# amorim-cleison/sign-language-nlp

Measured on AMD Instinct MI355X. Metric: train seq/s (batch=50,len=48), higher is better.
Workload: dtype bf16x3; 1 GPU; cfg2: Transformer train step E512 H8 N6 F512 batch 50 len 48 |src| 3000 |tgt| 202 dropout 0.1, fwd+CE+bwd+clip(0.5)+SGD(m=.9); launch=eager stream launches (auto: timed both in 9 untimed pre-warmup steps + warmup), per_gpu=independent fit (grid shard)

## Files before the change

sign-language-nlp_amd/csrc/attention.hip:

```cpp
#include "common.hpp"
#include "launch.hpp"

namespace slnlp {

constexpr int SMAX = 64;
constexpr int DCH = 64;
constexpr int TLD = 68;

typedef __attribute__((ext_vector_type(8))) __bf16 bf16x8;
typedef __attribute__((ext_vector_type(4))) short s16x4;
typedef __attribute__((ext_vector_type(8))) short s16x8;
typedef __attribute__((ext_vector_type(4))) float f32x4;

constexpr int ALD = 72;
constexpr int ATILE = SMAX * ALD;
constexpr int MFMA_DH = 64;

__device__ __forceinline__ void fetch_tile(const float* __restrict__ src, long ld, int B, int b, int S, int col0,
                                           int dc, int tid, float4 (&r)[4]) {
#pragma unroll
    for (int u = 0; u < 4; ++u) {
        const int idx = tid + 256 * u, s = idx >> 4, c = (idx & 15) << 2;
        const bool ok = s < S && c < dc;
        r[u] = *reinterpret_cast<const float4*>(src + ((long)(ok ? s : 0) * B + b) * ld + col0 + (ok ? c : 0));
// ... 27 lines not shown
    const s16x8 v = {v0[0], v0[1], v0[2], v0[3], v1[0], v1[1], v1[2], v1[3]};
    return __builtin_bit_cast(bf16x8, v);
}
__device__ __forceinline__ f32x4 mfma3(bf16x8 ah, bf16x8 al, bf16x8 bh, bf16x8 bl, f32x4 c) {
    c = __builtin_amdgcn_mfma_f32_16x16x32_bf16(al, bh, c, 0, 0, 0);
    c = __builtin_amdgcn_mfma_f32_16x16x32_bf16(ah, bl, c, 0, 0, 0);
    return __builtin_amdgcn_mfma_f32_16x16x32_bf16(ah, bh, c, 0, 0, 0);
}
__device__ __forceinline__ unsigned keep_mask8(const DropKey& key, unsigned row0, unsigned col, unsigned thr) {
    unsigned m = 0;
    if ((row0 & 3u) == 0u) {
        const uint4 bits = dropout_bits8(key, row0 >> 2, drop_cc(col));
#pragma unroll
        for (int h = 0; h < 2; ++h)
#pragma unroll
            for (int r = 0; r < 4; ++r) m |= (pick_lot(bits, h, r) >= thr ? 1u : 0u) << (4 * h + r);
    } else {
#pragma unroll
        for (int h = 0; h < 2; ++h)
#pragma unroll
            for (int r = 0; r < 4; ++r) m |= (dropout_keep(key, row0 + r, col + 16 * h, thr) ? 1u : 0u) << (4 * h + r);
    }
    return m;
}
__device__ __forceinline__ void put_planes(unsigned short* __restrict__ T, int off, float v) {
    unsigned short h, l;
    split_bf16(v, h, l);
    T[off] = h;
    T[ATILE + off] = l;
}

__device__ __forceinline__ void store_rows_via_lds(unsigned short* __restrict__ T, const f32x4 (&o)[4], int wave, int lane, int S, int dc,
                                                   const PlaneOut& po, long row_stride, long col0, int B, int b) {
    const int jc = lane & 15, i0 = wave * 16 + ((lane >> 4) << 2);
#pragma unroll
    for (int n = 0; n < 4; ++n)
#pragma unroll
        for (int r = 0; r < 4; ++r) put_planes(T, (i0 + r) * ALD + 16 * n + jc, o[n][r]);
    asm volatile("s_waitcnt lgkmcnt(0)" ::: "memory");
    __builtin_amdgcn_wave_barrier();
#pragma unroll
    for (int pass = 0; pass < 2; ++pass) {
        const int row = wave * 16 + pass * 8 + (lane >> 3), c8 = (lane & 7) << 3;
        if (row < S && c8 < dc) {
            const uint4 vh = *reinterpret_cast<const uint4*>(T + row * ALD + c8), vl = *reinterpret_cast<const uint4*>(T + ATILE + row * ALD + c8);
            const long at = ((long)row * B + b) * row_stride + col0 + c8;
// ... 139 lines not shown
    const unsigned long long* __restrict__ rng, PlaneOut po) {
    extern __shared__ __attribute__((aligned(16))) float smem[];
    unsigned short* TQ = reinterpret_cast<unsigned short*>(smem);
    unsigned short* TK = TQ + 2 * ATILE;
    unsigned short* TO = TQ + 4 * ATILE;
    unsigned short* TV = TQ + 6 * ATILE;
    const int tid = threadIdx.x, lane = tid & 63, wave = tid >> 6;
    const int b = blockIdx.x / H, h = blockIdx.x % H, E = H * dh;
    const long ld = 3L * E;
    const int jc = lane & 15, i0 = wave * 16 + ((lane >> 4) << 2);
    const long prow0 = ((long)b * H + h) * S + i0;
    const int nch = (dh + MFMA_DH - 1) / MFMA_DH;
    unsigned short* TS = nch > 1 ? TQ + 8 * ATILE : TO;

    float pr[4][4];
#pragma unroll
    for (int n = 0; n < 4; ++n)
#pragma unroll
        for (int r = 0; r < 4; ++r) {
            const int j = 16 * n + jc;
            const bool ok = (i0 + r) < S && j < S;
            pr[n][r] = probs[ok ? (prow0 + r) * S + j : 0];
        }
    f32x4 acc[4];
#pragma unroll
    for (int n = 0; n < 4; ++n) acc[n] = f32x4{0.f, 0.f, 0.f, 0.f};
    float4 rq[4], rk[4];
    for (int ch = 0; ch < nch; ++ch) {
        const int d0 = ch * MFMA_DH, dc = dh - d0 < MFMA_DH ? dh - d0 : MFMA_DH;
        float4 ro[4], rv[4];
        fetch_tile(dctx, E, B, b, S, h * dh + d0, dc, tid, ro);
        fetch_tile(qkv, ld, B, b, S, 2 * E + h * dh + d0, dc, tid, rv);
        if (nch == 1) {
            fetch_tile(qkv, ld, B, b, S, h * dh, dc, tid, rq);
            fetch_tile(qkv, ld, B, b, S, E + h * dh, dc, tid, rk);
        }
        if (ch > 0) __syncthreads();
        stash_tile(TO, S, dc, tid, ro);
        stash_tile(TV, S, dc, tid, rv);
        __syncthreads();
        const int nk = (dc + 31) >> 5;
        for (int kk = 0; kk < nk; ++kk) {
            const bf16x8 ah = frag_rows(TO, wave * 16, kk, lane), al = frag_rows(TO + ATILE, wave * 16, kk, lane);
#pragma unroll
            for (int n = 0; n < 4; ++n)
                acc[n] = mfma3(ah, al, frag_rows(TV, 16 * n, kk, lane), frag_rows(TV + ATILE, 16 * n, kk, lane), acc[n]);
        }
    }
    if (nch == 1) {
        stash_tile(TQ, S, dh, tid, rq);
        stash_tile(TK, S, dh, tid, rk);
    }
    const float scale = rsqrtf((float)dh), inv_keep = 1.f / (1.f - drop_p);
    float ds[4][4], pd[4][4];
    {
        unsigned keep[4] = {15u, 15u, 15u, 15u};
        if (drop_p > 0.f) {
            const DropKey dkey = dropout_key(rng, drop_site);
#pragma unroll
            for (int np = 0; np < 2; ++np) {
                if (32 * np + jc >= S || i0 >= S) continue;
                const unsigned m = keep_mask8(dkey, (unsigned)prow0, (unsigned)(32 * np + jc), drop_thr);
                keep[2 * np] = m & 15u;
                keep[2 * np + 1] = m >> 4;
            }
        }
#pragma unroll
        for (int r = 0; r < 4; ++r) {
            float dp[4], s = 0.f;
#pragma unroll
            for (int n = 0; n < 4; ++n) {
                const bool ok = (i0 + r) < S && (16 * n + jc) < S;
                const float p = ok ? pr[n][r] : 0.f;
                const bool k = (keep[n] >> r) & 1u;
                pr[n][r] = p;
                dp[n] = drop_p > 0.f ? (k ? acc[n][r] * inv_keep : 0.f) : acc[n][r];
                pd[n][r] = drop_p > 0.f ? (k ? p * inv_keep : 0.f) : p;
                s += dp[n] * p;
            }
            s = row16_sum(s);
#pragma unroll
            for (int n = 0; n < 4; ++n) ds[n][r] = pr[n][r] * (dp[n] - s) * scale;
        }
    }
    __syncthreads();
#pragma unroll
    for (int n = 0; n < 4; ++n)
#pragma unroll
        for (int r = 0; r < 4; ++r) {
// ... 363 lines not shown
```

sign-language-nlp_amd/csrc/attention_mem.hip:

```cpp
#include <stddef.h>

#include "common.hpp"
#include "launch.hpp"

namespace slnlp {


__device__ __forceinline__ int xcd_local(int i, int nb) { return (nb & 7) == 0 ? (i & 7) * (nb >> 3) + (i >> 3) : i; }

template <class F>
__device__ __forceinline__ void row_dots(const float* __restrict__ v, const float* __restrict__ mem, int B, int b, int S, int E, int lane,
                                         int wave, F&& put) {
    for (int s0 = wave; s0 < S; s0 += 16) {
        float a[4] = {0.f, 0.f, 0.f, 0.f};
#pragma unroll
        for (int u = 0; u < 4; ++u) {
            const int s = s0 + 4 * u;
            if (s < S) {
                const float* mr = mem + ((long)s * B + b) * E;
                for (int e = lane * 4; e < E; e += 256) {
                    const float4 m4 = *reinterpret_cast<const float4*>(mr + e), q4 = *reinterpret_cast<const float4*>(v + e);
                    a[u] += q4.x * m4.x + q4.y * m4.y + q4.z * m4.z + q4.w * m4.w;
                }
            }
        }
#pragma unroll
        for (int u = 0; u < 4; ++u) {
            const float r = wave_sum(a[u]);
            if (lane == 0 && s0 + 4 * u < S) put(s0 + 4 * u, r);
        }
    }
}

__device__ __forceinline__ void xmem_fwd_body(const float* __restrict__ qk, const float* __restrict__ mem, const float* __restrict__ bv,
                                              int B, int S, int H, int dh, float* __restrict__ mbar_out, float* __restrict__ psum_out,
                                              float* __restrict__ probs, float* __restrict__ ctx0, float drop_p, unsigned drop_thr,
                                              int drop_site, const unsigned long long* __restrict__ rng) {
    extern __shared__ __attribute__((aligned(16))) float xm_lds[];
    const int tid = threadIdx.x, lane = tid & 63, wave = tid >> 6;
    const int bh = xcd_local(blockIdx.x, gridDim.x), b = bh / H, h = bh % H, E = H * dh;
    float* qv = xm_lds;
    float* sc = qv + E;
    float* ps = sc + S;
    for (int e = tid * 4; e < E; e += 1024) *reinterpret_cast<float4*>(qv + e) = *reinterpret_cast<const float4*>(qk + (long)bh * E + e);
    __syncthreads();
    const float scale = rsqrtf((float)dh), inv_keep = 1.f / (1.f - drop_p);
    row_dots(qv, mem, B, b, S, E, lane, wave, [&](int s_, float r) { sc[s_] = r * scale; });
    __syncthreads();
    if (wave == 0) {
        float m = -INFINITY;
        for (int s = lane; s < S; s += 64) m = fmaxf(m, sc[s]);
        m = wave_max(m);
        float sum = 0.f;
        for (int s = lane; s < S; s += 64) sum += expf(sc[s] - m);
        sum = wave_sum(sum);
        float tot = 0.f;
        for (int s = lane; s < S; s += 64) {
            float p = expf(sc[s] - m) / sum;
            probs[(long)bh * S + s] = p;
            if (drop_p > 0.f) p = dropout_keep(rng, drop_site, (unsigned)bh, (unsigned)s, drop_thr) ? p * inv_keep : 0.f;
            sc[s] = p;
            tot += p;
        }
        tot = wave_sum(tot);
        if (lane == 0) {
            ps[0] = tot;
            psum_out[bh] = tot;
        }
    }
    __syncthreads();
    for (int e = tid * 4; e < E; e += 1024) {
        float4 a = make_float4(0.f, 0.f, 0.f, 0.f);
#pragma unroll 16
        for (int s = 0; s < S; ++s) {
            const float p = sc[s];
            const float4 m4 = *reinterpret_cast<const float4*>(mem + ((long)s * B + b) * E + e);
            a.x += p * m4.x; a.y += p * m4.y; a.z += p * m4.z; a.w += p * m4.w;
        }
        *reinterpret_cast<float4*>(mbar_out + (long)bh * E + e) = a;
    }
    for (int j = tid; j < dh; j += 256) ctx0[(long)b * E + h * dh + j] = bv[h * dh + j] * ps[0];
}
SLNLP_ZKERNEL(xmem_fwd_kernel, 256, xmem_fwd_body)

__device__ __forceinline__ void xmem_bwd_body(const float* __restrict__ mem, const float* __restrict__ bv, const float* __restrict__ probs,
                                              const float* __restrict__ psum, const float* __restrict__ dmbar,
                                              const float* __restrict__ dctx, int B, int S, int H, int dh, float* __restrict__ dsc_out,
                                              float* __restrict__ dqk_out, float* __restrict__ dcp, float drop_p, unsigned drop_thr,
                                              int drop_site, const unsigned long long* __restrict__ rng) {
    extern __shared__ __attribute__((aligned(16))) float xm_lds[];
    const int tid = threadIdx.x, lane = tid & 63, wave = tid >> 6;
    const int bh = xcd_local(blockIdx.x, gridDim.x), b = bh / H, h = bh % H, E = H * dh;
    float* dmb = xm_lds;
    float* t = dmb + E;
    float* cc = t + S;
    const float ps = psum[bh];
    for (int e = tid * 4; e < E; e += 1024) *reinterpret_cast<float4*>(dmb + e) = *reinterpret_cast<const float4*>(dmbar + (long)bh * E + e);
    if (wave == 0) {
        float c = 0.f;
        for (int j = lane; j < dh; j += 64) {
            const float g = dctx[(long)b * E + h * dh + j];
            c += g * bv[h * dh + j];
            dcp[(long)b * E + h * dh + j] = g * ps;
        }
        c = wave_sum(c);
        if (lane == 0) cc[0] = c;
    }
    __syncthreads();
    row_dots(dmb, mem, B, b, S, E, lane, wave, [&](int s_, float r) { t[s_] = r + cc[0]; });
    __syncthreads();
    const float scale = rsqrtf((float)dh), inv_keep = 1.f / (1.f - drop_p);
    if (wave == 0) {
        float dot = 0.f;
        for (int s = lane; s < S; s += 64) {
            float dp = t[s];
            if (drop_p > 0.f) dp = dropout_keep(rng, drop_site, (unsigned)bh, (unsigned)s, drop_thr) ? dp * inv_keep : 0.f;
            t[s] = dp;
            dot += probs[(long)bh * S + s] * dp;
        }
        dot = wave_sum(dot);
        for (int s = lane; s < S; s += 64) {
            const float v = probs[(long)bh * S + s] * (t[s] - dot) * scale;
            t[s] = v;
            dsc_out[(long)bh * S + s] = v;
        }
    }
    __syncthreads();
    for (int e = tid * 4; e < E; e += 1024) {
        float4 a = make_float4(0.f, 0.f, 0.f, 0.f);
#pragma unroll 16
        for (int s = 0; s < S; ++s) {
            const float w = t[s];
            const float4 m4 = *reinterpret_cast<const float4*>(mem + ((long)s * B + b) * E + e);
            a.x += w * m4.x; a.y += w * m4.y; a.z += w * m4.z; a.w += w * m4.w;
        }
        *reinterpret_cast<float4*>(dqk_out + (long)bh * E + e) = a;
    }
}
SLNLP_ZKERNEL(xmem_bwd_kernel, 256, xmem_bwd_body)

constexpr int XMEM_MAX_HEADS = 64;

constexpr int DMEM_ROWS = 8;
__device__ __forceinline__ void dmem_stage(const float* __restrict__ probs, const float* __restrict__ dsc, int b, int h, int s_, int S, int H,
                                           float drop_p, unsigned drop_thr, int drop_site, const unsigned long long* __restrict__ rng,
                                           float& p, float& d) {
    const long bh = (long)b * H + h;
    p = 0.f;
    d = 0.f;
    if (s_ < S) {
        p = probs[bh * S + s_];
        if (drop_p > 0.f) p = dropout_keep(rng, drop_site, (unsigned)bh, (unsigned)s_, drop_thr) ? p / (1.f - drop_p) : 0.f;
        d = dsc[bh * S + s_];
    }
}
constexpr int DMEM_HEADS = 2;
__device__ __forceinline__ void dmem_add_heads(float4 (&a)[DMEM_ROWS], const float* __restrict__ dmbar, const float* __restrict__ qk,
                                               const float* ph, const float* dh_, int ld, int b, int H, int E, int e, int set, int sets) {
    const int ni = (DMEM_ROWS + sets - 1) / sets;
    for (int h0 = 0; h0 < H; h0 += DMEM_HEADS) {
        float4 g[DMEM_HEADS], k[DMEM_HEADS];
#pragma unroll
        for (int u = 0; u < DMEM_HEADS; ++u) {
            const long bh = (long)b * H + (h0 + u < H ? h0 + u : H - 1);
            g[u] = *reinterpret_cast<const float4*>(dmbar + bh * E + e);
            k[u] = *reinterpret_cast<const float4*>(qk + bh * E + e);
        }
#pragma unroll
        for (int u = 0; u < DMEM_HEADS; ++u) {
            if (h0 + u >= H) break;
#pragma unroll
            for (int i = 0; i < DMEM_ROWS; ++i) {
                if (i >= ni) break;
                const int r = set + i * sets;
                const bool ok = r < DMEM_ROWS;
                const float p = ok ? ph[r * ld + h0 + u] : 0.f, d = ok ? dh_[r * ld + h0 + u] : 0.f;
                a[i].x += p * g[u].x + d * k[u].x; a[i].y += p * g[u].y + d * k[u].y; a[i].z += p * g[u].z + d * k[u].z; a[i].w += p * g[u].w + d * k[u].w;
            }
        }
    }
}
__device__ __forceinline__ void dmem_colsum(const float* __restrict__ dcp, int B, int E, int c, float* __restrict__ dbv) {
    if (c >= E) return;
    float a = 0.f;
#pragma unroll 8
    for (int r = 0; r < B; ++r) a += dcp[(long)r * E + c];
    dbv[c] = a;
}

__device__ __forceinline__ void xmem_dmem_body(const float* __restrict__ probs, const float* __restrict__ dsc, const float* __restrict__ dmbar,
                                               const float* __restrict__ qk, int B, int S, int H, int E, float* __restrict__ dmem,
                                               int accumulate, float drop_p, unsigned drop_thr, int drop_site,
                                               const unsigned long long* __restrict__ rng, const float* __restrict__ dcp,
                                               float* __restrict__ dbv) {
    __shared__ float ph[DMEM_ROWS][XMEM_MAX_HEADS], dh_[DMEM_ROWS][XMEM_MAX_HEADS];
    const int chunks = (S + DMEM_ROWS - 1) / DMEM_ROWS, tid = threadIdx.x;
    if ((int)blockIdx.x >= chunks * B) {
        dmem_colsum(dcp, B, E, ((int)blockIdx.x - chunks * B) * 256 + tid, dbv);
        return;
    }
    const int b = blockIdx.x / chunks, s0 = (blockIdx.x % chunks) * DMEM_ROWS;
    for (int i = tid; i < DMEM_ROWS * H; i += 256) {
        const int r = i / H, h = i - r * H;
        float p, d;
        dmem_stage(probs, dsc, b, h, s0 + r, S, H, drop_p, drop_thr, drop_site, rng, p, d);
        ph[r][h] = p;
        dh_[r][h] = d;
    }
    __syncthreads();
    const int per = E >> 2, sets = per >= 256 ? 1 : 256 / per;
    const int set = sets == 1 ? 0 : tid / per, c0 = sets == 1 ? tid : tid - set * per;
    if (set >= sets) return;
    for (int e = c0 * 4; e < E; e += (sets == 1 ? 1024 : E)) {
        float4 a[DMEM_ROWS];
#pragma unroll
        for (int i = 0; i < DMEM_ROWS; ++i) {
            const int r = set + i * sets, s_ = s0 + r;
            a[i] = make_float4(0.f, 0.f, 0.f, 0.f);
            if (accumulate && r < DMEM_ROWS && s_ < S) a[i] = *reinterpret_cast<const float4*>(dmem + ((long)s_ * B + b) * E + e);
        }
        dmem_add_heads(a, dmbar, qk, &ph[0][0], &dh_[0][0], XMEM_MAX_HEADS, b, H, E, e, set, sets);
#pragma unroll
        for (int i = 0; i < DMEM_ROWS; ++i) {
            const int r = set + i * sets, s_ = s0 + r;
            if (r < DMEM_ROWS && s_ < S) *reinterpret_cast<float4*>(dmem + ((long)s_ * B + b) * E + e) = a[i];
        }
    }
}
SLNLP_ZKERNEL(xmem_dmem_kernel, 256, xmem_dmem_body)

constexpr int DMEM_STAGE_LAYERS = 8;
template <class T>
__device__ __forceinline__ T* dmem_ptr(T* p) {
    const unsigned long long v = (unsigned long long)p;
    const unsigned lo = __builtin_amdgcn_readfirstlane((unsigned)v), hi = __builtin_amdgcn_readfirstlane((unsigned)(v >> 32));
    return as_global((T*)(((unsigned long long)hi << 32) | lo));
}
__device__ __forceinline__ void xmem_dmem_all_body(const XmemDmemLayer* __restrict__ tab, int N, int B, int S, int H, int E,
                                                   float* __restrict__ dmem, float drop_p, unsigned drop_thr,
                                                   const unsigned long long* __restrict__ rng) {
    extern __shared__ __attribute__((aligned(16))) float xm_lds[];
    const int chunks = (S + DMEM_ROWS - 1) / DMEM_ROWS, tid = threadIdx.x;
    if ((int)blockIdx.x >= chunks * B) {
        const int cb = (E + 255) / 256, i = (int)blockIdx.x - chunks * B, l = i / cb;
        if (l < N) dmem_colsum(dmem_ptr(tab[l].dcp), B, E, (i - l * cb) * 256 + tid, dmem_ptr(tab[l].dbv));
        return;
    }
    const int b = blockIdx.x / chunks, s0 = (blockIdx.x % chunks) * DMEM_ROWS;
    const int per = E >> 2, sets = per >= 256 ? 1 : 256 / per;
    const int set = sets == 1 ? 0 : tid / per, c0 = sets == 1 ? tid : tid - set * per, e = c0 * 4;
    const bool active = set < sets && e < E;
    const int lf = DMEM_ROWS * H, wave = __builtin_amdgcn_readfirstlane(tid >> 6), lane = tid & 63;
    float4 a[DMEM_ROWS];
#pragma unroll
    for (int i = 0; i < DMEM_ROWS; ++i) a[i] = make_float4(0.f, 0.f, 0.f, 0.f);
    for (int l1 = N; l1 > 0; l1 -= DMEM_STAGE_LAYERS) {
        const int n = l1 < DMEM_STAGE_LAYERS ? l1 : DMEM_STAGE_LAYERS;
        if (l1 != N) __syncthreads();
        for (int j = wave; j < n; j += 4) {
            const XmemDmemLayer L = tab[l1 - 1 - j];
            const float* __restrict__ probs = dmem_ptr(L.probs);
            const float* __restrict__ dsc = dmem_ptr(L.dsc);
            for (int i = lane; i < lf; i += 64) {
                const int r = i / H, h = i - r * H;
                float p, d;
                dmem_stage(probs, dsc, b, h, s0 + r, S, H, drop_p, drop_thr, L.drop_site, rng, p, d);
                xm_lds[2 * j * lf + i] = p;
                xm_lds[(2 * j + 1) * lf + i] = d;
            }
        }
        __syncthreads();
        if (active)
            for (int j = 0; j < n; ++j) {
                const XmemDmemLayer L = tab[l1 - 1 - j];
                dmem_add_heads(a, dmem_ptr(L.dmbar), dmem_ptr(L.qk), xm_lds + 2 * j * lf, xm_lds + (2 * j + 1) * lf, H, b, H, E, e, set, sets);
            }
    }
    if (!active) return;
#pragma unroll
    for (int i = 0; i < DMEM_ROWS; ++i) {
        const int r = set + i * sets, s_ = s0 + r;
        if (r < DMEM_ROWS && s_ < S) *reinterpret_cast<float4*>(dmem + ((long)s_ * B + b) * E + e) = a[i];
    }
}
SLNLP_ZKERNEL(xmem_dmem_all_kernel, 256, xmem_dmem_all_body)

__device__ __forceinline__ void xmem_colsum_body(const float* __restrict__ in, int R, int C, float* __restrict__ out) {
    const int c = blockIdx.x * 256 + threadIdx.x;
    if (c >= C) return;
// ... 33 lines not shown
#pragma unroll
        for (int u = 0; u < RU; ++u)
#pragma unroll
            for (int hp = 0; hp < HP; ++hp) {
                const float r = wave_sum(a[u][hp]);
                if (lane == 0 && s0 + 4 * u < S) put(hp, s0 + 4 * u, r);
            }
    }
}

__device__ __forceinline__ int xm_head_floats(int S, int E) { return E + ((S + 3) & ~3) + 4; }

template <int HP>
__device__ __forceinline__ void xmem_fwd_multi_body(const float* __restrict__ qk, const float* __restrict__ mem, const float* __restrict__ bv,
                                                    int B, int S, int H, int dh, float* __restrict__ mbar_out, float* __restrict__ psum_out,
                                                    float* __restrict__ probs, float* __restrict__ ctx0, float drop_p, unsigned drop_thr,
                                                    int drop_site, const unsigned long long* __restrict__ rng) {
    extern __shared__ __attribute__((aligned(16))) float xm_lds[];
    const int tid = threadIdx.x, lane = tid & 63, wave = tid >> 6;
    const int E = H * dh, groups = H / HP;
    const int wg = xcd_local(blockIdx.x, gridDim.x), b = wg / groups, h0 = (wg % groups) * HP;
    const int hf = xm_head_floats(S, E), sp = (S + 3) & ~3;
    float* heads = xm_lds;
    for (int i = tid * 4; i < HP * E; i += 1024) {
        const int hp = i / E, e = i - hp * E;
        *reinterpret_cast<float4*>(heads + (long)hp * hf + e) = *reinterpret_cast<const float4*>(qk + ((long)b * H + h0 + hp) * E + e);
    }
    __syncthreads();
    const float scale = rsqrtf((float)dh), inv_keep = 1.f / (1.f - drop_p);
    row_dots_multi<HP>(heads, hf, mem, B, b, S, E, lane, wave, [&](int hp, int s_, float r) { heads[(long)hp * hf + E + s_] = r * scale; });
    __syncthreads();
    for (int hp = wave; hp < HP; hp += 4) {
        float* sc = heads + (long)hp * hf + E;
        const long bh = (long)b * H + h0 + hp;
        float m = -INFINITY;
        for (int s_ = lane; s_ < S; s_ += 64) m = fmaxf(m, sc[s_]);
        m = wave_max(m);
        float sum = 0.f;
        for (int s_ = lane; s_ < S; s_ += 64) sum += expf(sc[s_] - m);
        sum = wave_sum(sum);
        float tot = 0.f;
        for (int s_ = lane; s_ < S; s_ += 64) {
            float p = expf(sc[s_] - m) / sum;
            probs[bh * S + s_] = p;
            if (drop_p > 0.f) p = dropout_keep(rng, drop_site, (unsigned)bh, (unsigned)s_, drop_thr) ? p * inv_keep : 0.f;
            sc[s_] = p;
            tot += p;
        }
        tot = wave_sum(tot);
        if (lane == 0) {
            sc[sp] = tot;
            psum_out[bh] = tot;
        }
    }
    __syncthreads();
    for (int e = tid * 4; e < E; e += 1024) {
        float4 a[HP];
#pragma unroll
        for (int hp = 0; hp < HP; ++hp) a[hp] = make_float4(0.f, 0.f, 0.f, 0.f);
#pragma unroll 8
        for (int s_ = 0; s_ < S; ++s_) {
            const float4 m4 = *reinterpret_cast<const float4*>(mem + ((long)s_ * B + b) * E + e);
#pragma unroll
            for (int hp = 0; hp < HP; ++hp) {
                const float p = heads[(long)hp * hf + E + s_];
                a[hp].x += p * m4.x; a[hp].y += p * m4.y; a[hp].z += p * m4.z; a[hp].w += p * m4.w;
            }
        }
// ... 10 lines not shown
                                                 const unsigned long long* rng) {
    xmem_fwd_multi_body<2>(qk, mem, bv, B, S, H, dh, mbar_out, psum_out, probs, ctx0, drop_p, drop_thr, drop_site, rng);
}
__device__ __forceinline__ void xmem_fwd_h4_body(const float* qk, const float* mem, const float* bv, int B, int S, int H, int dh, float* mbar_out,
                                                 float* psum_out, float* probs, float* ctx0, float drop_p, unsigned drop_thr, int drop_site,
                                                 const unsigned long long* rng) {
    xmem_fwd_multi_body<4>(qk, mem, bv, B, S, H, dh, mbar_out, psum_out, probs, ctx0, drop_p, drop_thr, drop_site, rng);
}
SLNLP_ZKERNEL(xmem_fwd_h2_kernel, 256, xmem_fwd_h2_body)
SLNLP_ZKERNEL(xmem_fwd_h4_kernel, 256, xmem_fwd_h4_body)

template <int HP>
__device__ __forceinline__ void xmem_bwd_multi_body(const float* __restrict__ mem, const float* __restrict__ bv, const float* __restrict__ probs,
                                                    const float* __restrict__ psum, const float* __restrict__ dmbar,
                                                    const float* __restrict__ dctx, int B, int S, int H, int dh, float* __restrict__ dsc_out,
                                                    float* __restrict__ dqk_out, float* __restrict__ dcp, float drop_p, unsigned drop_thr,
                                                    int drop_site, const unsigned long long* __restrict__ rng) {
    extern __shared__ __attribute__((aligned(16))) float xm_lds[];
    const int tid = threadIdx.x, lane = tid & 63, wave = tid >> 6;
    const int E = H * dh, groups = H / HP;
    const int wg = xcd_local(blockIdx.x, gridDim.x), b = wg / groups, h0 = (wg % groups) * HP;
    const int hf = xm_head_floats(S, E), sp = (S + 3) & ~3;
    float* heads = xm_lds;
    for (int i = tid * 4; i < HP * E; i += 1024) {
        const int hp = i / E, e = i - hp * E;
        *reinterpret_cast<float4*>(heads + (long)hp * hf + e) = *reinterpret_cast<const float4*>(dmbar + ((long)b * H + h0 + hp) * E + e);
    }
    for (int hp = wave; hp < HP; hp += 4) {
        const int h = h0 + hp;
        const float ps = psum[(long)b * H + h];
        float c = 0.f;
        for (int j = lane; j < dh; j += 64) {
            const float g = dctx[(long)b * E + h * dh + j];
            c += g * bv[h * dh + j];
            dcp[(long)b * E + h * dh + j] = g * ps;
        }
        c = wave_sum(c);
        if (lane == 0) heads[(long)hp * hf + E + sp] = c;
    }
    __syncthreads();
    row_dots_multi<HP>(heads, hf, mem, B, b, S, E, lane, wave,
                       [&](int hp, int s_, float r) { heads[(long)hp * hf + E + s_] = r + heads[(long)hp * hf + E + sp]; });
    __syncthreads();
    const float scale = rsqrtf((float)dh), inv_keep = 1.f / (1.f - drop_p);
    for (int hp = wave; hp < HP; hp += 4) {
        float* t = heads + (long)hp * hf + E;
        const long bh = (long)b * H + h0 + hp;
        float dot = 0.f;
        for (int s_ = lane; s_ < S; s_ += 64) {
            float dp = t[s_];
            if (drop_p > 0.f) dp = dropout_keep(rng, drop_site, (unsigned)bh, (unsigned)s_, drop_thr) ? dp * inv_keep : 0.f;
            t[s_] = dp;
            dot += probs[bh * S + s_] * dp;
        }
        dot = wave_sum(dot);
        for (int s_ = lane; s_ < S; s_ += 64) {
            const float v = probs[bh * S + s_] * (t[s_] - dot) * scale;
            t[s_] = v;
            dsc_out[bh * S + s_] = v;
        }
    }
    __syncthreads();
    for (int e = tid * 4; e < E; e += 1024) {
        float4 a[HP];
#pragma unroll
        for (int hp = 0; hp < HP; ++hp) a[hp] = make_float4(0.f, 0.f, 0.f, 0.f);
#pragma unroll 8
        for (int s_ = 0; s_ < S; ++s_) {
            const float4 m4 = *reinterpret_cast<const float4*>(mem + ((long)s_ * B + b) * E + e);
#pragma unroll
            for (int hp = 0; hp < HP; ++hp) {
                const float w = heads[(long)hp * hf + E + s_];
                a[hp].x += w * m4.x; a[hp].y += w * m4.y; a[hp].z += w * m4.z; a[hp].w += w * m4.w;
            }
        }
#pragma unroll
        for (int hp = 0; hp < HP; ++hp) *reinterpret_cast<float4*>(dqk_out + ((long)b * H + h0 + hp) * E + e) = a[hp];
    }
}
__device__ __forceinline__ void xmem_bwd_h2_body(const float* mem, const float* bv, const float* probs, const float* psum, const float* dmbar,
                                                 const float* dctx, int B, int S, int H, int dh, float* dsc_out, float* dqk_out, float* dcp,
                                                 float drop_p, unsigned drop_thr, int drop_site, const unsigned long long* rng) {
    xmem_bwd_multi_body<2>(mem, bv, probs, psum, dmbar, dctx, B, S, H, dh, dsc_out, dqk_out, dcp, drop_p, drop_thr, drop_site, rng);
}
// ... 130 lines not shown
```

sign-language-nlp_amd/csrc/elementwise.hip:

```cpp
#include "common.hpp"
#include "launch.hpp"
#include "layernorm_row.hpp"

namespace slnlp {

__device__ __forceinline__ void embed_fwd_body(const long* __restrict__ ids, long ld_ids, int B, int S,
                                                        int E, int V, const float* __restrict__ table,
                                                        const float* __restrict__ pe, float* __restrict__ out,
                                                        float scale, float drop_p, unsigned drop_thr, int drop_site,
                                                        const unsigned long long* __restrict__ rng, long nan_idx,
                                                        PlaneOut po, unsigned char* __restrict__ keep_mask) {
    const int e4 = E >> 2;
    const long total = (long)B * S * e4;
    const float ik = 1.f / (1.f - drop_p);
    for (long idx = blockIdx.x * 256L + threadIdx.x; idx < total; idx += (long)gridDim.x * 256) {
        const int m = (int)(idx / e4), c = (int)(idx % e4) * 4;
        const int s = m / B, b = m % B;
        const long id = ids[(long)b * ld_ids + s];
        float4 v = make_float4(0.f, 0.f, 0.f, 0.f);
        if (id >= 0 && id < V) v = *reinterpret_cast<const float4*>(table + id * E + c);
        const float4 p = pe ? *reinterpret_cast<const float4*>(pe + (long)s * E + c) : make_float4(0.f, 0.f, 0.f, 0.f);
        v.x = v.x * scale + p.x; v.y = v.y * scale + p.y; v.z = v.z * scale + p.z; v.w = v.w * scale + p.w;
        if (drop_p > 0.f) {
            const bool k0 = dropout_keep(rng, drop_site, m, c + 0, drop_thr), k1 = dropout_keep(rng, drop_site, m, c + 1, drop_thr);
// ... 295 lines not shown
    const float* __restrict__ dy, const float* __restrict__ x, const float* __restrict__ gamma,
    const float* __restrict__ stats, int rows, int E, const float* __restrict__ add_to_dx, float* __restrict__ dx,
    float* __restrict__ dx_drop, float drop_p, unsigned drop_thr, int drop_site,
    const unsigned long long* __restrict__ rng, PlaneOut po_dx, PlaneOut po_drop, float* __restrict__ partial, int chunk_rows, int nchunks) {
    const int lane = threadIdx.x & 63, wave = threadIdx.x >> 6;
    const float invE = 1.f / (float)E, ik = 1.f / (1.f - drop_p);
    const bool want_drop = dx_drop != nullptr || po_drop.hi != nullptr;
    const bool drop = want_drop && drop_p > 0.f;
    const int unit = FUSE ? (int)blockIdx.x : blockIdx.x * (int)(blockDim.x >> 6) + wave;
    float4 ag[U], ab[U];
#pragma unroll
    for (int u = 0; u < U; ++u) ag[u] = ab[u] = make_float4(0.f, 0.f, 0.f, 0.f);
    const int row_begin = FUSE ? unit * chunk_rows + wave * GS : unit * GS;
    const int row_end = FUSE ? ((unit + 1) * chunk_rows < rows ? (unit + 1) * chunk_rows : rows) : row_begin + GS;
    const int row_step = FUSE ? 4 * GS : GS;
    if (!FUSE && row_begin >= rows) return;
    DropKey dkey = {};
    if (drop) dkey = dropout_key(rng, drop_site);
    float4 g[U];
#pragma unroll
    for (int u = 0; u < U; ++u)
        if (lane * 4 + u * 256 < E) g[u] = *reinterpret_cast<const float4*>(gamma + lane * 4 + u * 256);
#pragma unroll 1
    for (int row0 = row_begin; row0 < row_end; row0 += row_step)
#pragma unroll
    for (int i0 = 0; i0 < GS; i0 += RB) {
        float4 d[RB][U], v[RB][U];
        float mean[RB], rstd[RB], s1[RB], s2[RB];
#pragma unroll
        for (int i = 0; i < RB; ++i) {
            const int row = row0 + i0 + i < rows ? row0 + i0 + i : rows - 1;
            mean[i] = stats[2 * row];
            rstd[i] = stats[2 * row + 1];
#pragma unroll
            for (int u = 0; u < U; ++u) {
                const int c = lane * 4 + u * 256;
                if (c < E) {
                    d[i][u] = *reinterpret_cast<const float4*>(dy + (long)row * E + c);
                    v[i][u] = *reinterpret_cast<const float4*>(x + (long)row * E + c);
                }
            }
        }
#pragma unroll
        for (int i = 0; i < RB; ++i) {
            float a1 = 0.f, a2 = 0.f;
#pragma unroll
            for (int u = 0; u < U; ++u) {
                if (lane * 4 + u * 256 < E) {
                    const float4 dd = d[i][u], vv = v[i][u];
                    const float4 xh = make_float4((vv.x - mean[i]) * rstd[i], (vv.y - mean[i]) * rstd[i], (vv.z - mean[i]) * rstd[i], (vv.w - mean[i]) * rstd[i]);
                    const float4 gv = make_float4(dd.x * g[u].x, dd.y * g[u].y, dd.z * g[u].z, dd.w * g[u].w);
                    a1 += gv.x + gv.y + gv.z + gv.w;
                    a2 += gv.x * xh.x + gv.y * xh.y + gv.z * xh.z + gv.w * xh.w;
                }
            }
            s1[i] = wave_sum(a1) * invE;
            s2[i] = wave_sum(a2) * invE;
        }
#pragma unroll
        for (int u = 0; u < U; ++u) {
            const int c = lane * 4 + u * 256;
            if (c >= E) continue;
            uint4 kb[4];
            const int half = drop_half((unsigned)c);
            if (drop) {
#pragma unroll
                for (int e = 0; e < 4; ++e) kb[e] = dropout_bits8(dkey, (unsigned)(row0 + i0) >> 2, drop_cc((unsigned)(c + e)));
            }
#pragma unroll
            for (int i = 0; i < RB; ++i) {
                const int row = row0 + i0 + i;
                if (row >= rows) continue;
                const int wsel = row & 3;
                const float4 dd = d[i][u], vv = v[i][u];
                const float4 xh = make_float4((vv.x - mean[i]) * rstd[i], (vv.y - mean[i]) * rstd[i], (vv.z - mean[i]) * rstd[i], (vv.w - mean[i]) * rstd[i]);
                const float4 gv = make_float4(dd.x * g[u].x, dd.y * g[u].y, dd.z * g[u].z, dd.w * g[u].w);
                if (FUSE) {
                    ag[u].x += dd.x * xh.x; ag[u].y += dd.y * xh.y; ag[u].z += dd.z * xh.z; ag[u].w += dd.w * xh.w;
                    ab[u].x += dd.x; ab[u].y += dd.y; ab[u].z += dd.z; ab[u].w += dd.w;
                }
                float4 o;
                o.x = rstd[i] * (gv.x - s1[i] - xh.x * s2[i]); o.y = rstd[i] * (gv.y - s1[i] - xh.y * s2[i]);
                o.z = rstd[i] * (gv.z - s1[i] - xh.z * s2[i]); o.w = rstd[i] * (gv.w - s1[i] - xh.w * s2[i]);
                if (add_to_dx) {
                    const float4 a = *reinterpret_cast<const float4*>(add_to_dx + (long)row * E + c);
                    o.x += a.x; o.y += a.y; o.z += a.z; o.w += a.w;
                }
                *reinterpret_cast<float4*>(dx + (long)row * E + c) = o;
                store_planes4(po_dx, (long)row * E + c, o);
                if (want_drop) {
                    if (drop) {
                        o.x = pick_lot(kb[0], half, wsel) >= drop_thr ? o.x * ik : 0.f;
                        o.y = pick_lot(kb[1], half, wsel) >= drop_thr ? o.y * ik : 0.f;
                        o.z = pick_lot(kb[2], half, wsel) >= drop_thr ? o.z * ik : 0.f;
                        o.w = pick_lot(kb[3], half, wsel) >= drop_thr ? o.w * ik : 0.f;
                    }
                    if (dx_drop) *reinterpret_cast<float4*>(dx_drop + (long)row * E + c) = o;
                    store_planes4(po_drop, (long)row * E + c, o);
                }
            }
        }
    }
    if (FUSE) {
        __shared__ float4 red[4][2][U * 64];
#pragma unroll
        for (int u = 0; u < U; ++u) {
            red[wave][0][u * 64 + lane] = ag[u];
            red[wave][1][u * 64 + lane] = ab[u];
        }
        __syncthreads();
        for (int q = threadIdx.x; q < 2 * U * 64; q += 256) {
            const int which = q / (U * 64), slot = q - which * (U * 64), c = (slot & 63) * 4 + (slot >> 6) * 256;
            if (c >= E) continue;
            float4 t = red[0][which][slot];
#pragma unroll
            for (int k = 1; k < 4; ++k) {
                const float4 o = red[k][which][slot];
                t.x += o.x; t.y += o.y; t.z += o.z; t.w += o.w;
            }
            *reinterpret_cast<float4*>(partial + ((long)unit * 2 + which) * E + c) = t;
        }
    }
}

// ... 501 lines not shown
```

Baseline: 21920 seq/s.

## Precompute dropout keep masks early to overlap RNG with global loads

Moves dropout keep-bit generation in attention backward, cross-memory attention forward/backward and layernorm backward so it runs while global tile and vector loads are in flight. The RNG seed words are read through scalar constant address space and the keep decisions are packed into bitmasks up front. Per-head entry values (psum, dctx, bv, probs) are also prefetched during LDS staging. The intent is to hide the hash-based RNG ALU latency and shorten the serial softmax/dropout tail, at the cost of extra live registers and more intricate code.

```diff
diff --git a/sign-language-nlp_amd/csrc/attention.hip b/sign-language-nlp_amd/csrc/attention.hip
--- a/sign-language-nlp_amd/csrc/attention.hip
+++ b/sign-language-nlp_amd/csrc/attention.hip
@@ -73,6 +73,21 @@
             for (int r = 0; r < 4; ++r) m |= (dropout_keep(key, row0 + r, col + 16 * h, thr) ? 1u : 0u) << (4 * h + r);
     }
     return m;
+}
+typedef const __attribute__((address_space(4))) unsigned long long* const_words;
+__device__ __forceinline__ void self_keep_flags(unsigned long long seed, unsigned long long step, int drop_site, unsigned drop_thr, long prow0,
+                                                int jc, int S, unsigned (&keep)[4]) {
+    DropKey dkey = dropout_key(seed, step, drop_site);
+    asm volatile("" : "+s"(dkey.ks[0]) : : "memory");
+#pragma unroll
+    for (int np = 0; np < 2; ++np) {
+        if (32 * np + jc >= S) continue;
+        const unsigned m = keep_mask8(dkey, (unsigned)prow0, (unsigned)(32 * np + jc), drop_thr);
+        keep[2 * np] = m & 15u;
+        keep[2 * np + 1] = m >> 4;
+    }
+#pragma unroll
+    for (int n = 0; n < 4; ++n) asm volatile("" : "+v"(keep[n]));
 }
 __device__ __forceinline__ void put_planes(unsigned short* __restrict__ T, int off, float v) {
     unsigned short h, l;
@@ -258,6 +273,9 @@
             const bool ok = (i0 + r) < S && j < S;
             pr[n][r] = probs[ok ? (prow0 + r) * S + j : 0];
         }
+    unsigned keep[4] = {15u, 15u, 15u, 15u};
+    unsigned long long rseed = 0, rstep = 0;
+    if (drop_p > 0.f) { rseed = ((const_words)rng)[0]; rstep = ((const_words)rng)[1]; }
     f32x4 acc[4];
 #pragma unroll
     for (int n = 0; n < 4; ++n) acc[n] = f32x4{0.f, 0.f, 0.f, 0.f};
@@ -271,6 +289,7 @@
             fetch_tile(qkv, ld, B, b, S, h * dh, dc, tid, rq);
             fetch_tile(qkv, ld, B, b, S, E + h * dh, dc, tid, rk);
         }
+        if (ch == 0 && drop_p > 0.f && i0 < S) self_keep_flags(rseed, rstep, drop_site, drop_thr, prow0, jc, S, keep);
         if (ch > 0) __syncthreads();
         stash_tile(TO, S, dc, tid, ro);
         stash_tile(TV, S, dc, tid, rv);
@@ -290,17 +309,6 @@
     const float scale = rsqrtf((float)dh), inv_keep = 1.f / (1.f - drop_p);
     float ds[4][4], pd[4][4];
     {
-        unsigned keep[4] = {15u, 15u, 15u, 15u};
-        if (drop_p > 0.f) {
-            const DropKey dkey = dropout_key(rng, drop_site);
-#pragma unroll
-            for (int np = 0; np < 2; ++np) {
-                if (32 * np + jc >= S || i0 >= S) continue;
-                const unsigned m = keep_mask8(dkey, (unsigned)prow0, (unsigned)(32 * np + jc), drop_thr);
-                keep[2 * np] = m & 15u;
-                keep[2 * np + 1] = m >> 4;
-            }
-        }
 #pragma unroll
         for (int r = 0; r < 4; ++r) {
             float dp[4], s = 0.f;
diff --git a/sign-language-nlp_amd/csrc/attention_mem.hip b/sign-language-nlp_amd/csrc/attention_mem.hip
--- a/sign-language-nlp_amd/csrc/attention_mem.hip
+++ b/sign-language-nlp_amd/csrc/attention_mem.hip
@@ -30,6 +30,92 @@
             if (lane == 0 && s0 + 4 * u < S) put(s0 + 4 * u, r);
         }
     }
+}
+
+constexpr int XM_KEEP_TRIPS = 32;
+__device__ __forceinline__ unsigned xm_keep_bits(const unsigned long long* __restrict__ rng, int drop_site, unsigned drop_thr, long bh, int S, int lane,
+                                                 DropKey& key) {
+    typedef const __attribute__((address_space(4))) unsigned long long* const_words;
+    const const_words rw = (const_words)rng;
+    key = dropout_key(rw[0], rw[1], drop_site);
+    asm volatile("" : "+s"(key.ks[0]) : : "memory");
+    unsigned bits = 0;
+    int t = 0;
+    for (int s_ = lane; s_ < S && t < XM_KEEP_TRIPS; s_ += 64, ++t) bits |= (dropout_keep(key, (unsigned)bh, (unsigned)s_, drop_thr) ? 1u : 0u) << t;
+    asm volatile("" : "+v"(bits));
+    return bits;
+}
+__device__ __forceinline__ bool xm_keep(unsigned bits, int t, const DropKey& key, unsigned drop_thr, long bh, int s_) {
+    return t < XM_KEEP_TRIPS ? ((bits >> t) & 1u) != 0u : dropout_keep(key, (unsigned)bh, (unsigned)s_, drop_thr);
+}
+template <class F>
+__device__ __forceinline__ void xm_stage_vectors(float* __restrict__ dst, int hf, const float* __restrict__ src, int n, int E, int tid, F&& under) {
+    const int i0 = tid * 4;
+    const float4 first = *reinterpret_cast<const float4*>(src + (i0 < n ? i0 : 0));
+    under();
+    if (i0 < n) {
+        const int hp = i0 / E;
+        *reinterpret_cast<float4*>(dst + (long)hp * hf + (i0 - hp * E)) = first;
+    }
+    for (int i = i0 + 1024; i < n; i += 1024) {
+        const int hp = i / E;
+        *reinterpret_cast<float4*>(dst + (long)hp * hf + (i - hp * E)) = *reinterpret_cast<const float4*>(src + i);
+    }
+}
+constexpr int XM_PROB_TRIPS = 2;
+struct XmBwdEntry {
+    float ps, g0, bv0, pr[XM_PROB_TRIPS];
+};
+__device__ __forceinline__ XmBwdEntry xm_bwd_entry(const float* __restrict__ psum, const float* __restrict__ dctx, const float* __restrict__ bv,
+                                                   const float* __restrict__ probs, int b, int h, int H, int dh, int S, int lane) {
+    XmBwdEntry r;
+    const long bh = (long)b * H + h;
+    const int j = lane < dh ? lane : 0;
+    r.ps = psum[bh];
+    r.g0 = dctx[(long)b * H * dh + h * dh + j];
+    r.bv0 = bv[h * dh + j];
+#pragma unroll
+    for (int t = 0; t < XM_PROB_TRIPS; ++t) r.pr[t] = probs[bh * S + (lane + 64 * t < S ? lane + 64 * t : S - 1)];
+    return r;
+}
+__device__ __forceinline__ float xm_bwd_head_c(const XmBwdEntry& en, const float* __restrict__ dctx, const float* __restrict__ bv, float* __restrict__ dcp,
+                                               int b, int h, int E, int dh, int lane) {
+    float c = 0.f;
+    if (lane < dh) {
+        c += en.g0 * en.bv0;
+        dcp[(long)b * E + h * dh + lane] = en.g0 * en.ps;
+    }
+    for (int j = lane + 64; j < dh; j += 64) {
+        const float g = dctx[(long)b * E + h * dh + j];
+        c += g * bv[h * dh + j];
+        dcp[(long)b * E + h * dh + j] = g * en.ps;
+    }
+    return wave_sum(c);
+}
+__device__ __forceinline__ void xm_bwd_head_softmax(float* __restrict__ t, const XmBwdEntry& en, unsigned kbits, const float* __restrict__ probs,
+                                                    float* __restrict__ dsc_out, long bh, int S, int lane, float scale, float inv_keep, float drop_p,
+                                                    unsigned drop_thr, const DropKey& dkey) {
+    float dot = 0.f;
+    auto first = [&](int s_, int tr, float p) {
+        float dp = t[s_];
+        if (drop_p > 0.f) dp = xm_keep(kbits, tr, dkey, drop_thr, bh, s_) ? dp * inv_keep : 0.f;
+        t[s_] = dp;
+        dot += p * dp;
+    };
+#pragma unroll
+    for (int tr = 0; tr < XM_PROB_TRIPS; ++tr)
+        if (lane + 64 * tr < S) first(lane + 64 * tr, tr, en.pr[tr]);
+    for (int s_ = lane + 64 * XM_PROB_TRIPS, tr = XM_PROB_TRIPS; s_ < S; s_ += 64, ++tr) first(s_, tr, probs[bh * S + s_]);
+    dot = wave_sum(dot);
+    auto second = [&](int s_, float p) {
+        const float v = p * (t[s_] - dot) * scale;
+        t[s_] = v;
+        dsc_out[bh * S + s_] = v;
+    };
+#pragma unroll
+    for (int tr = 0; tr < XM_PROB_TRIPS; ++tr)
+        if (lane + 64 * tr < S) second(lane + 64 * tr, en.pr[tr]);
+    for (int s_ = lane + 64 * XM_PROB_TRIPS; s_ < S; s_ += 64) second(s_, probs[bh * S + s_]);
 }
 
 __device__ __forceinline__ void xmem_fwd_body(const float* __restrict__ qk, const float* __restrict__ mem, const float* __restrict__ bv,
@@ -42,7 +128,11 @@
     float* qv = xm_lds;
     float* sc = qv + E;
     float* ps = sc + S;
-    for (int e = tid * 4; e < E; e += 1024) *reinterpret_cast<float4*>(qv + e) = *reinterpret_cast<const float4*>(qk + (long)bh * E + e);
+    DropKey dkey = {};
+    unsigned kbits = 0;
+    xm_stage_vectors(qv, 0, qk + (long)bh * E, E, E, tid, [&] {
+        if (wave == 0 && drop_p > 0.f) kbits = xm_keep_bits(rng, drop_site, drop_thr, bh, S, lane, dkey);
+    });
     __syncthreads();
     const float scale = rsqrtf((float)dh), inv_keep = 1.f / (1.f - drop_p);
     row_dots(qv, mem, B, b, S, E, lane, wave, [&](int s_, float r) { sc[s_] = r * scale; });
@@ -55,10 +145,10 @@
         for (int s = lane; s < S; s += 64) sum += expf(sc[s] - m);
         sum = wave_sum(sum);
         float tot = 0.f;
-        for (int s = lane; s < S; s += 64) {
+        for (int s = lane, tr = 0; s < S; s += 64, ++tr) {
             float p = expf(sc[s] - m) / sum;
             probs[(long)bh * S + s] = p;
-            if (drop_p > 0.f) p = dropout_keep(rng, drop_site, (unsigned)bh, (unsigned)s, drop_thr) ? p * inv_keep : 0.f;
+            if (drop_p > 0.f) p = xm_keep(kbits, tr, dkey, drop_thr, bh, s) ? p * inv_keep : 0.f;
             sc[s] = p;
             tot += p;
         }
@@ -94,37 +184,22 @@
     float* dmb = xm_lds;
     float* t = dmb + E;
     float* cc = t + S;
-    const float ps = psum[bh];
-    for (int e = tid * 4; e < E; e += 1024) *reinterpret_cast<float4*>(dmb + e) = *reinterpret_cast<const float4*>(dmbar + (long)bh * E + e);
+    XmBwdEntry en;
+    DropKey dkey = {};
+    unsigned kbits = 0;
+    xm_stage_vectors(dmb, 0, dmbar + (long)bh * E, E, E, tid, [&] {
+        en = xm_bwd_entry(psum, dctx, bv, probs, b, h, H, dh, S, lane);
+        if (wave == 0 && drop_p > 0.f) kbits = xm_keep_bits(rng, drop_site, drop_thr, bh, S, lane, dkey);
+    });
     if (wave == 0) {
-        float c = 0.f;
-        for (int j = lane; j < dh; j += 64) {
-            const float g = dctx[(long)b * E + h * dh + j];
-            c += g * bv[h * dh + j];
-            dcp[(long)b * E + h * dh + j] = g * ps;
-        }
-        c = wave_sum(c);
+        const float c = xm_bwd_head_c(en, dctx, bv, dcp, b, h, E, dh, lane);
         if (lane == 0) cc[0] = c;
     }
     __syncthreads();
     row_dots(dmb, mem, B, b, S, E, lane, wave, [&](int s_, float r) { t[s_] = r + cc[0]; });
     __syncthreads();
     const float scale = rsqrtf((float)dh), inv_keep = 1.f / (1.f - drop_p);
-    if (wave == 0) {
-        float dot = 0.f;
-        for (int s = lane; s < S; s += 64) {
-            float dp = t[s];
-            if (drop_p > 0.f) dp = dropout_keep(rng, drop_site, (unsigned)bh, (unsigned)s, drop_thr) ? dp * inv_keep : 0.f;
-            t[s] = dp;
-            dot += probs[(long)bh * S + s] * dp;
-        }
-        dot = wave_sum(dot);
-        for (int s = lane; s < S; s += 64) {
-            const float v = probs[(long)bh * S + s] * (t[s] - dot) * scale;
-            t[s] = v;
-            dsc_out[(long)bh * S + s] = v;
-        }
-    }
+    if (wave == 0) xm_bwd_head_softmax(t, en, kbits, probs, dsc_out, bh, S, lane, scale, inv_keep, drop_p, drop_thr, dkey);
     __syncthreads();
     for (int e = tid * 4; e < E; e += 1024) {
         float4 a = make_float4(0.f, 0.f, 0.f, 0.f);
@@ -142,16 +217,25 @@
 constexpr int XMEM_MAX_HEADS = 64;
 
 constexpr int DMEM_ROWS = 8;
+__device__ __forceinline__ void dmem_rng_words(const unsigned long long* __restrict__ rng, float drop_p, unsigned long long& seed, unsigned long long& step) {
+    typedef const __attribute__((address_space(4))) unsigned long long* const_words;
+    seed = step = 0;
+    if (drop_p > 0.f) { seed = ((const_words)rng)[0]; step = ((const_words)rng)[1]; }
+}
 __device__ __forceinline__ void dmem_stage(const float* __restrict__ probs, const float* __restrict__ dsc, int b, int h, int s_, int S, int H,
-                                           float drop_p, unsigned drop_thr, int drop_site, const unsigned long long* __restrict__ rng,
+                                           float drop_p, unsigned drop_thr, int drop_site, unsigned long long seed, unsigned long long step,
                                            float& p, float& d) {
     const long bh = (long)b * H + h;
     p = 0.f;
     d = 0.f;
     if (s_ < S) {
         p = probs[bh * S + s_];
-        if (drop_p > 0.f) p = dropout_keep(rng, drop_site, (unsigned)bh, (unsigned)s_, drop_thr) ? p / (1.f - drop_p) : 0.f;
         d = dsc[bh * S + s_];
+        if (drop_p > 0.f) {
+            unsigned keep = dropout_keep(dropout_key(seed, step, drop_site), (unsigned)bh, (unsigned)s_, drop_thr) ? 1u : 0u;
+            asm volatile("" : "+v"(keep), "+v"(p));
+            p = keep ? p / (1.f - drop_p) : 0.f;
+        }
     }
 }
 constexpr int DMEM_HEADS = 2;
@@ -195,6 +279,8 @@
                                                float* __restrict__ dbv) {
     __shared__ float ph[DMEM_ROWS][XMEM_MAX_HEADS], dh_[DMEM_ROWS][XMEM_MAX_HEADS];
     const int chunks = (S + DMEM_ROWS - 1) / DMEM_ROWS, tid = threadIdx.x;
+    unsigned long long seed, step;
+    dmem_rng_words(rng, drop_p, seed, step);
     if ((int)blockIdx.x >= chunks * B) {
         dmem_colsum(dcp, B, E, ((int)blockIdx.x - chunks * B) * 256 + tid, dbv);
         return;
@@ -203,7 +289,7 @@
     for (int i = tid; i < DMEM_ROWS * H; i += 256) {
         const int r = i / H, h = i - r * H;
         float p, d;
-        dmem_stage(probs, dsc, b, h, s0 + r, S, H, drop_p, drop_thr, drop_site, rng, p, d);
+        dmem_stage(probs, dsc, b, h, s0 + r, S, H, drop_p, drop_thr, drop_site, seed, step, p, d);
         ph[r][h] = p;
         dh_[r][h] = d;
     }
@@ -241,6 +327,8 @@
                                                    const unsigned long long* __restrict__ rng) {
     extern __shared__ __attribute__((aligned(16))) float xm_lds[];
     const int chunks = (S + DMEM_ROWS - 1) / DMEM_ROWS, tid = threadIdx.x;
+    unsigned long long seed, step;
+    dmem_rng_words(rng, drop_p, seed, step);
     if ((int)blockIdx.x >= chunks * B) {
         const int cb = (E + 255) / 256, i = (int)blockIdx.x - chunks * B, l = i / cb;
         if (l < N) dmem_colsum(dmem_ptr(tab[l].dcp), B, E, (i - l * cb) * 256 + tid, dmem_ptr(tab[l].dbv));
@@ -264,7 +352,7 @@
             for (int i = lane; i < lf; i += 64) {
                 const int r = i / H, h = i - r * H;
                 float p, d;
-                dmem_stage(probs, dsc, b, h, s0 + r, S, H, drop_p, drop_thr, L.drop_site, rng, p, d);
+                dmem_stage(probs, dsc, b, h, s0 + r, S, H, drop_p, drop_thr, L.drop_site, seed, step, p, d);
                 xm_lds[2 * j * lf + i] = p;
                 xm_lds[(2 * j + 1) * lf + i] = d;
             }
@@ -344,10 +432,12 @@
     const int wg = xcd_local(blockIdx.x, gridDim.x), b = wg / groups, h0 = (wg % groups) * HP;
     const int hf = xm_head_floats(S, E), sp = (S + 3) & ~3;
     float* heads = xm_lds;
-    for (int i = tid * 4; i < HP * E; i += 1024) {
-        const int hp = i / E, e = i - hp * E;
-        *reinterpret_cast<float4*>(heads + (long)hp * hf + e) = *reinterpret_cast<const float4*>(qk + ((long)b * H + h0 + hp) * E + e);
-    }
+    static_assert(HP <= 4, "a wave owns at most one head: head hp is wave hp's");
+    DropKey dkey = {};
+    unsigned kbits = 0;
+    xm_stage_vectors(heads, hf, qk + ((long)b * H + h0) * E, HP * E, E, tid, [&] {
+        if (wave < HP && drop_p > 0.f) kbits = xm_keep_bits(rng, drop_site, drop_thr, (long)b * H + h0 + wave, S, lane, dkey);
+    });
     __syncthreads();
     const float scale = rsqrtf((float)dh), inv_keep = 1.f / (1.f - drop_p);
     row_dots_multi<HP>(heads, hf, mem, B, b, S, E, lane, wave, [&](int hp, int s_, float r) { heads[(long)hp * hf + E + s_] = r * scale; });
@@ -362,10 +452,10 @@
         for (int s_ = lane; s_ < S; s_ += 64) sum += expf(sc[s_] - m);
         sum = wave_sum(sum);
         float tot = 0.f;
-        for (int s_ = lane; s_ < S; s_ += 64) {
+        for (int s_ = lane, tr = 0; s_ < S; s_ += 64, ++tr) {
             float p = expf(sc[s_] - m) / sum;
             probs[bh * S + s_] = p;
-            if (drop_p > 0.f) p = dropout_keep(rng, drop_site, (unsigned)bh, (unsigned)s_, drop_thr) ? p * inv_keep : 0.f;
+            if (drop_p > 0.f) p = xm_keep(kbits, tr, dkey, drop_thr, bh, s_) ? p * inv_keep : 0.f;
             sc[s_] = p;
             tot += p;
         }
@@ -422,20 +512,17 @@
     const int wg = xcd_local(blockIdx.x, gridDim.x), b = wg / groups, h0 = (wg % groups) * HP;
     const int hf = xm_head_floats(S, E), sp = (S + 3) & ~3;
     float* heads = xm_lds;
-    for (int i = tid * 4; i < HP * E; i += 1024) {
-        const int hp = i / E, e = i - hp * E;
-        *reinterpret_cast<float4*>(heads + (long)hp * hf + e) = *reinterpret_cast<const float4*>(dmbar + ((long)b * H + h0 + hp) * E + e);
-    }
+    static_assert(HP <= 4, "a wave owns at most one head: head hp is wave hp's");
+    const int hown = h0 + (wave < HP ? wave : 0);
+    XmBwdEntry en;
+    DropKey dkey = {};
+    unsigned kbits = 0;
+    xm_stage_vectors(heads, hf, dmbar + ((long)b * H + h0) * E, HP * E, E, tid, [&] {
+        en = xm_bwd_entry(psum, dctx, bv, probs, b, hown, H, dh, S, lane);
+        if (wave < HP && drop_p > 0.f) kbits = xm_keep_bits(rng, drop_site, drop_thr, (long)b * H + hown, S, lane, dkey);
+    });
     for (int hp = wave; hp < HP; hp += 4) {
-        const int h = h0 + hp;
-        const float ps = psum[(long)b * H + h];
-        float c = 0.f;
-        for (int j = lane; j < dh; j += 64) {
-            const float g = dctx[(long)b * E + h * dh + j];
-            c += g * bv[h * dh + j];
-            dcp[(long)b * E + h * dh + j] = g * ps;
-        }
-        c = wave_sum(c);
+        const float c = xm_bwd_head_c(en, dctx, bv, dcp, b, h0 + hp, E, dh, lane);
         if (lane == 0) heads[(long)hp * hf + E + sp] = c;
     }
     __syncthreads();
@@ -443,23 +530,9 @@
                        [&](int hp, int s_, float r) { heads[(long)hp * hf + E + s_] = r + heads[(long)hp * hf + E + sp]; });
     __syncthreads();
     const float scale = rsqrtf((float)dh), inv_keep = 1.f / (1.f - drop_p);
-    for (int hp = wave; hp < HP; hp += 4) {
-        float* t = heads + (long)hp * hf + E;
-        const long bh = (long)b * H + h0 + hp;
-        float dot = 0.f;
-        for (int s_ = lane; s_ < S; s_ += 64) {
-            float dp = t[s_];
-            if (drop_p > 0.f) dp = dropout_keep(rng, drop_site, (unsigned)bh, (unsigned)s_, drop_thr) ? dp * inv_keep : 0.f;
-            t[s_] = dp;
-            dot += probs[bh * S + s_] * dp;
-        }
-        dot = wave_sum(dot);
-        for (int s_ = lane; s_ < S; s_ += 64) {
-            const float v = probs[bh * S + s_] * (t[s_] - dot) * scale;
-            t[s_] = v;
-            dsc_out[bh * S + s_] = v;
-        }
-    }
+    for (int hp = wave; hp < HP; hp += 4)
+        xm_bwd_head_softmax(heads + (long)hp * hf + E, en, kbits, probs, dsc_out, (long)b * H + h0 + hp, S, lane, scale, inv_keep, drop_p, drop_thr,
+                            dkey);
     __syncthreads();
     for (int e = tid * 4; e < E; e += 1024) {
         float4 a[HP];
diff --git a/sign-language-nlp_amd/csrc/elementwise.hip b/sign-language-nlp_amd/csrc/elementwise.hip
--- a/sign-language-nlp_amd/csrc/elementwise.hip
+++ b/sign-language-nlp_amd/csrc/elementwise.hip
@@ -341,7 +341,10 @@
     for (int u = 0; u < U; ++u)
         if (lane * 4 + u * 256 < E) g[u] = *reinterpret_cast<const float4*>(gamma + lane * 4 + u * 256);
 #pragma unroll 1
-    for (int row0 = row_begin; row0 < row_end; row0 += row_step)
+    for (int row0 = row_begin; row0 < row_end; row0 += row_step) {
+    unsigned kp[U];
+#pragma unroll
+    for (int u = 0; u < U; ++u) kp[u] = 0u;
 #pragma unroll
     for (int i0 = 0; i0 < GS; i0 += RB) {
         float4 d[RB][U], v[RB][U];
@@ -358,6 +361,21 @@
                     d[i][u] = *reinterpret_cast<const float4*>(dy + (long)row * E + c);
                     v[i][u] = *reinterpret_cast<const float4*>(x + (long)row * E + c);
                 }
+            }
+        }
+        if (i0 == 0 && drop) {
+#pragma unroll
+            for (int u = 0; u < U; ++u) {
+                const int c = lane * 4 + u * 256;
+                const int half = drop_half((unsigned)c);
+#pragma unroll
+                for (int e = 0; e < 4; ++e) {
+                    const uint4 kb = dropout_bits8(dkey, (unsigned)row0 >> 2, drop_cc((unsigned)(c + e)));
+#pragma unroll
+                    for (int i = 0; i < GS; ++i)
+                        kp[u] |= (pick_lot(kb, half, (row0 + i) & 3) >= drop_thr ? 1u : 0u) << (4 * i + e);
+                }
+                asm volatile("" : "+v"(kp[u]));
             }
         }
 #pragma unroll
@@ -380,17 +398,11 @@
         for (int u = 0; u < U; ++u) {
             const int c = lane * 4 + u * 256;
             if (c >= E) continue;
-            uint4 kb[4];
-            const int half = drop_half((unsigned)c);
-            if (drop) {
-#pragma unroll
-                for (int e = 0; e < 4; ++e) kb[e] = dropout_bits8(dkey, (unsigned)(row0 + i0) >> 2, drop_cc((unsigned)(c + e)));
-            }
 #pragma unroll
             for (int i = 0; i < RB; ++i) {
                 const int row = row0 + i0 + i;
                 if (row >= rows) continue;
-                const int wsel = row & 3;
+                const unsigned k4 = kp[u] >> (4 * (i0 + i));
                 const float4 dd = d[i][u], vv = v[i][u];
                 const float4 xh = make_float4((vv.x - mean[i]) * rstd[i], (vv.y - mean[i]) * rstd[i], (vv.z - mean[i]) * rstd[i], (vv.w - mean[i]) * rstd[i]);
                 const float4 gv = make_float4(dd.x * g[u].x, dd.y * g[u].y, dd.z * g[u].z, dd.w * g[u].w);
@@ -409,16 +421,17 @@
                 store_planes4(po_dx, (long)row * E + c, o);
                 if (want_drop) {
                     if (drop) {
-                        o.x = pick_lot(kb[0], half, wsel) >= drop_thr ? o.x * ik : 0.f;
-                        o.y = pick_lot(kb[1], half, wsel) >= drop_thr ? o.y * ik : 0.f;
-                        o.z = pick_lot(kb[2], half, wsel) >= drop_thr ? o.z * ik : 0.f;
-                        o.w = pick_lot(kb[3], half, wsel) >= drop_thr ? o.w * ik : 0.f;
+                        o.x = (k4 & 1u) ? o.x * ik : 0.f;
+                        o.y = (k4 & 2u) ? o.y * ik : 0.f;
+                        o.z = (k4 & 4u) ? o.z * ik : 0.f;
+                        o.w = (k4 & 8u) ? o.w * ik : 0.f;
                     }
                     if (dx_drop) *reinterpret_cast<float4*>(dx_drop + (long)row * E + c) = o;
                     store_planes4(po_drop, (long)row * E + c, o);
                 }
             }
         }
+    }
     }
     if (FUSE) {
         __shared__ float4 red[4][2][U * 64];
```

Result: no change. 22030 seq/s (median of 6 runs) (+0.5%).
